# harukaki/brl

Measured on AMD Instinct MI355X. Metric: env-steps/sec at num_envs=8192, 32-step rollout, 1/2/4/8 MI355X, higher is better.
Workload: dtype u8

## Files before the change

brl_amd/csrc/brl_ppo.hip:

```cpp
#include <hip/hip_runtime.h>
#include <math.h>
#include <stdint.h>
#include <stdio.h>
#include <stdlib.h>
#include <string.h>

#include "abi_common.hpp"

static inline unsigned thread_grid(int64_t n, int bs) { return (unsigned)((n + bs - 1) / bs); }

struct PpoArgs {
  const float *logits;
  int64_t ls;
  const float *value;
  const uint8_t *mask;
  const int32_t *action;
  const float *old_value, *old_logp, *gae, *tgt;
  int64_t B;
  float clip_eps, vf_coef, ent_coef;
  int masked, value_clipping;
  float *dlogits, *dvalue, *partials, *illp;
  int64_t vs, dls, dvs;
};

// ... 297 lines not shown
  return BRL_OK;
}

#ifdef FAIR_TIMING
extern "C" int brl_fair_set_dbg(void *p) {
  HIP_TRY(hipMemcpyToSymbol(HIP_SYMBOL(g_fair_dbg), &p, sizeof(p)));
  return BRL_OK;
}
#endif

extern "C" int brl_fair_chain(int device, const brl_fair_net *net, const float *x0, const uint8_t *mask, const int32_t *action,
                              const float *old_value, const float *old_log_prob, const float *gae, const float *targets,
                              int64_t batch, float clip_eps, float vf_coef, float ent_coef, int masked, int value_clipping,
                              int reward_scaling, int act, const brl_fair_work *work, void *stream) {
  NEED(net && work && x0 && mask && action && old_value && old_log_prob && gae && targets, "NULL input");
  NEED(batch > 0 && batch % fair::R == 0, "batch (a multiple of 16)");
  NEED(act == 0 || act == 1, "act");
  fair::Args A{};
  for (int l = 0; l < 11; l++) {
    NEED(net->w[l] && net->b[l], "net: NULL layer");
    NEED((((uintptr_t)net->w[l]) & 15) == 0 && (((uintptr_t)net->b[l]) & 15) == 0, "net: 16-byte alignment");
    A.net.w[l] = net->w[l]; A.net.b[l] = net->b[l];
  }
  NEED(net->head_w && net->head_b && (((uintptr_t)net->head_w) & 15) == 0, "net: heads");
  A.net.wh = net->head_w; A.net.bh = net->head_b;
  NEED(work->inp && work->dzs && work->gates && work->cat6 && work->x4 && work->dz0 && work->dz6 && work->dheads && work->tiles &&
       work->partials, "work: NULL array");
  const void *al[] = {x0, work->inp, work->dzs, work->gates, work->cat6, work->x4, work->dz0, work->dz6, work->tiles};
  for (const void *q : al) NEED((((uintptr_t)q) & 15) == 0, "16-byte alignment");
  A.o = fair::Bufs{work->inp, work->dzs, work->gates, work->cat6, work->x4, work->dz0, work->dz6, work->dheads, work->tiles,
                   work->partials, work->gram_partials};
  A.x0 = x0;
  A.P = PpoArgs{nullptr, 0, nullptr, mask, action, old_value, old_log_prob, gae, targets, batch, clip_eps, vf_coef,
                ent_coef, masked, value_clipping, nullptr, nullptr, nullptr, nullptr, 1, BRL_NUM_ACTIONS, 1};
  A.act = act;
  A.reward_scaling = reward_scaling;
  HIP_TRY(hipSetDevice(device));
  A.nrows = batch;
  hipLaunchKernelGGL(fair::k_fair_chain<true>, dim3((unsigned)(batch / fair::R)), dim3(fair::NW * 64), 0, (hipStream_t)stream, A);
  HIP_TRY(hipGetLastError());
  return BRL_OK;
}

extern "C" int brl_fair_forward(int device, const brl_fair_net *net, const float *x, int64_t rows, int act, float *logits, float *value,
                                void *stream) {
  NEED(net && x && logits && value, "NULL array");
  NEED(rows >= 0 && rows < (1ll << 31), "rows");
  NEED(act == 0 || act == 1, "act");
  if (rows == 0) return BRL_OK;
  fair::Args A{};
  for (int l = 0; l < 11; l++) {
    NEED(net->w[l] && net->b[l], "net: NULL layer");
    NEED((((uintptr_t)net->w[l]) & 15) == 0 && (((uintptr_t)net->b[l]) & 15) == 0, "net: 16-byte alignment");
    A.net.w[l] = net->w[l]; A.net.b[l] = net->b[l];
  }
  NEED(net->head_w && net->head_b && (((uintptr_t)net->head_w) & 15) == 0 && (((uintptr_t)x) & 15) == 0, "net: heads / x: 16-byte alignment");
  A.net.wh = net->head_w; A.net.bh = net->head_b;
  A.x0 = x;
  A.act = act;
  A.nrows = rows;
  A.logits_out = logits;
  A.value_out = value;
  HIP_TRY(hipSetDevice(device));
  hipLaunchKernelGGL(fair::k_fair_chain<false>, dim3((unsigned)((rows + fair::R - 1) / fair::R)), dim3(fair::NW * 64), 0,
                     (hipStream_t)stream, A);
  HIP_TRY(hipGetLastError());
  return BRL_OK;
}

extern "C" int brl_ppo_heads_loss_split(int device, const float *h, int64_t ldh, const float *head_w, const float *head_b,
                                        int64_t hidden, const uint8_t *mask, const int32_t *action, const float *old_value,
                                        const float *old_log_prob, const float *gae, const float *targets, int64_t batch,
                                        float clip_eps, float vf_coef, float ent_coef, int masked, int value_clipping,
                                        int reward_scaling, float *heads_out, float *dheads, float *partials, float *gram_partials,
                                        float *head_parts, int ksplit, void *stream) {
  NEED(batch > 0 && hidden > 0 && hidden % 16 == 0 && ldh >= hidden && ldh % 4 == 0, "batch / hidden (a multiple of 16) / ldh");
  NEED(h && head_w && head_b && mask && action && old_value && old_log_prob && gae && targets, "NULL input array");
  NEED(dheads && partials && head_parts, "NULL output array");
  NEED(ksplit >= 1 && ksplit <= 8, "ksplit (1..8)");
// ... 170 lines not shown
```

brl_amd/csrc/fair_chain.hpp:

```cpp
#pragma once

#ifndef FAIR_EXP
#define FAIR_EXP 0
#endif
#ifdef FAIR_TIMING
__device__ unsigned long long *g_fair_dbg = nullptr;
#define FAIR_STAMP(k) do { if (threadIdx.x == 0 && g_fair_dbg) g_fair_dbg[(size_t)blockIdx.x * 64 + (k)] = __builtin_amdgcn_s_memtime(); } while (0)
#else
#define FAIR_STAMP(k) do { } while (0)
#endif
namespace fair {
constexpr int H = 200, OBS = 480, CAT = 680;
constexpr int R = 16;
constexpr int NW = 8;
constexpr int NT = 13;
constexpr int LDA = 208;
constexpr int LDX = 484;
constexpr int LDH = 48;
typedef float f32x4 __attribute__((ext_vector_type(4)));

struct Net {
  const float *w[11], *b[11];
  const float *wh, *bh;
};
struct Bufs {
  float *inp, *dzs, *gates, *cat6, *x4, *dz0, *dz6, *dheads, *tiles, *partials, *gram_partials;
};
struct Args {
// ... 12 lines not shown
__device__ __forceinline__ f32x4 act4(f32x4 v, int act) {
  if (act == 0) return f32x4{fmaxf(v.x, 0.f), fmaxf(v.y, 0.f), fmaxf(v.z, 0.f), fmaxf(v.w, 0.f)};
  return f32x4{tanhf(v.x), tanhf(v.y), tanhf(v.z), tanhf(v.w)};
}
__device__ __forceinline__ f32x4 dact4(f32x4 d, f32x4 h, int act) {
  if (act == 0) return f32x4{h.x > 0.f ? d.x : 0.f, h.y > 0.f ? d.y : 0.f, h.z > 0.f ? d.z : 0.f, h.w > 0.f ? d.w : 0.f};
  return f32x4{d.x * (1.f - h.x * h.x), d.y * (1.f - h.y * h.y), d.z * (1.f - h.z * h.z), d.w * (1.f - h.w * h.w)};
}
__device__ __forceinline__ float row16_sum(float v) {
  v += dpp_move_f<0xB1>(0.0f, v);
  v += dpp_move_f<0x4E>(0.0f, v);
  v += dpp_move_f<0x124>(0.0f, v);
  v += dpp_move_f<0x128>(0.0f, v);
  return v;
}
__device__ __forceinline__ f32x4 row16_sum4(f32x4 v) { return f32x4{row16_sum(v.x), row16_sum(v.y), row16_sum(v.z), row16_sum(v.w)}; }

constexpr int FCH = 15;
struct Frag { f32x4 w[FCH]; };
struct Job {
  const float *W;
  int ldw, nch, nn, n0, nmax;
  int real;
};

struct JobAddr {
  __amdgpu_buffer_rsrc_t rs;
  int voff, vtail;
  int nn, wide, nch;
};
__device__ __forceinline__ JobAddr job_addr(const Job &J, const int c, const int g) {
// ... 19 lines not shown
  if ((FAIR_EXP & 64) && !a.nn) return;
  if (!a.nn) {
    if (j == 12) F.w[j] = __builtin_bit_cast(f32x4, __builtin_amdgcn_raw_buffer_load_b128(a.rs, a.vtail, 0, 0));
    else F.w[j] = __builtin_bit_cast(f32x4, __builtin_amdgcn_raw_buffer_load_b128(a.rs, a.voff, 64 * j, 0));
  } else {
    const int v = (j == 12) ? a.vtail : a.voff;
    if (!a.wide) {
#pragma unroll
      for (int s = 0; s < 4; s++) F.w[j][s] = __builtin_bit_cast(float, __builtin_amdgcn_raw_buffer_load_b32(a.rs, v, (16 * j + s) * H * 4, 0));
    } else {
#pragma unroll
      for (int s = 0; s < 4; s++) F.w[j][s] = __builtin_bit_cast(float, __builtin_amdgcn_raw_buffer_load_b32(a.rs, v, (16 * j + s) * CAT * 4, 0));
    }
  }
}
template <int j>
__device__ __forceinline__ void mac_chunk(f32x4 &acc, const Frag &F, const f32x4 &xv) {
#pragma unroll
  for (int s = 0; s < 4; s++) {
    if (FAIR_EXP & 1) acc[s] += F.w[j][s] * xv[s];
    else acc = __builtin_amdgcn_mfma_f32_16x16x4f32(F.w[j][s], xv[s], acc, 0, 0, 0);
  }
}
template <int j>
__device__ __forceinline__ void slot_step(f32x4 &acc, const Frag &use, Frag &pre, const JobAddr &na, const int nch, const float *xrow,
                                          f32x4 &xv) {
  f32x4 xn = xv;
  if (!(FAIR_EXP & 4) && (j + 1 < 13 || (j + 1 < FCH && nch > 13))) xn = ld4(xrow + 16 * (j + 1));
  if (j < 13 || na.nch > 13) load_chunk<j>(pre, na);
  if (j < 13 || nch > 13) mac_chunk<j>(acc, use, xv);
  __builtin_amdgcn_sched_barrier(0);
  xv = xn;
}
__device__ __forceinline__ void slot_run(f32x4 &acc, const Frag &use, Frag &pre, const Job &cur, const Job &nxt, const float *X,
                                         const int ldx, const int c, const int g, const int gs) {
  const JobAddr na = job_addr(nxt, c, g);
  const float *xrow = X + c * ldx + 4 * (ldx == LDA ? gs : g);
  const int nch = cur.nch;
  f32x4 xv = (FAIR_EXP & 4) ? f32x4{1.f, 1.f, 1.f, 1.f} : ld4(xrow);
  __builtin_amdgcn_sched_barrier(0);
  slot_step<0>(acc, use, pre, na, nch, xrow, xv);
  slot_step<1>(acc, use, pre, na, nch, xrow, xv);
  slot_step<2>(acc, use, pre, na, nch, xrow, xv);
  slot_step<3>(acc, use, pre, na, nch, xrow, xv);
  slot_step<4>(acc, use, pre, na, nch, xrow, xv);
  slot_step<5>(acc, use, pre, na, nch, xrow, xv);
  slot_step<6>(acc, use, pre, na, nch, xrow, xv);
  slot_step<7>(acc, use, pre, na, nch, xrow, xv);
  slot_step<8>(acc, use, pre, na, nch, xrow, xv);
  slot_step<9>(acc, use, pre, na, nch, xrow, xv);
  slot_step<10>(acc, use, pre, na, nch, xrow, xv);
  slot_step<11>(acc, use, pre, na, nch, xrow, xv);
  slot_step<12>(acc, use, pre, na, nch, xrow, xv);
  if (nch > 13 || na.nch > 13) {
    slot_step<13>(acc, use, pre, na, nch, xrow, xv);
    slot_step<14>(acc, use, pre, na, nch, xrow, xv);
  }
}
__device__ __forceinline__ void load_job(Frag &F, const Job &J, const int c, const int g) {
  const JobAddr a = job_addr(J, c, g);
  load_chunk<0>(F, a); load_chunk<1>(F, a); load_chunk<2>(F, a); load_chunk<3>(F, a); load_chunk<4>(F, a); load_chunk<5>(F, a);
  load_chunk<6>(F, a); load_chunk<7>(F, a); load_chunk<8>(F, a); load_chunk<9>(F, a); load_chunk<10>(F, a); load_chunk<11>(F, a);
  load_chunk<12>(F, a);
  if (a.nch > 13) { load_chunk<13>(F, a); load_chunk<14>(F, a); }
}

template <bool TRAIN>
__global__ __launch_bounds__(NW * 64) void k_fair_chain(Args A) {
  __shared__ __attribute__((aligned(16))) float X0[R * LDX];
  __shared__ __attribute__((aligned(16))) float AB[3][R * LDA];
  __shared__ __attribute__((aligned(16))) float HD[R * LDH], DH[TRAIN ? R * LDH : 4];
  __shared__ float illp_s[TRAIN ? R : 1][BRL_NUM_ACTIONS], part_s[TRAIN ? R : 1][8];
  __shared__ float rs_red[NW], rs_stat[2];
  const int tid = (int)threadIdx.x, lane = tid & 63, c = lane & 15, g = lane >> 4;
  const int gs = g ^ ((0x78 >> (2 * (c >> 2))) & 3);
  const int sw4 = 4 * (gs - g);
  const int w = __builtin_amdgcn_readfirstlane(tid >> 6);
  const int64_t B = TRAIN ? A.P.B : A.nrows, row0 = (int64_t)blockIdx.x * R, nwg = gridDim.x;
  const int act = A.act;
  const Net &N = A.net;
  const Bufs &O = A.o;
  const int64_t BH = B * H;
  float *const a0 = AB[0], *const a1 = AB[1], *const a2 = AB[2];

  const bool hasA = w < 7, hasB = w < 6;
  const int tA = hasA ? 32 * w : 0, tB = hasB ? tA + 16 : tA;
  auto job_fwd = [&](const float *W, int ldw, int nch, bool B) { return Job{W, ldw, nch, 0, B ? tB : tA, H, (B ? hasB : hasA) ? 1 : 0}; };
  auto job_bwd = [&](const float *W, int ldw, bool B) { return Job{W, ldw, 13, 1, B ? tB : tA, H, (B ? hasB : hasA) ? 1 : 0}; };
  Frag FP, FQ;
  int stamp_i = 0;
  (void)stamp_i;
  FAIR_STAMP(stamp_i++);
  constexpr int XP = (R * (OBS / 4) + NW * 64 - 1) / (NW * 64);
  f32x4 xv[XP];
#pragma unroll
  for (int i = 0; i < XP; i++) {
    const int e = tid + i * NW * 64, ec = (e < R * (OBS / 4)) ? e : 0;
    const int r = ec / (OBS / 4), q = ec - r * (OBS / 4);
// ... 37 lines not shown
    q = wave_sum_f(q);
    __syncthreads();
    if (lane == 0) rs_red[w] = q;
    __syncthreads();
    if (tid == 0) {
      float t = 0.0f;
      for (int k = 0; k < NW; k++) t += rs_red[k];
      rs_stat[1] = 1.0f / (sqrtf(t / (float)B) + 1e-8f);
    }
    __syncthreads();
    adv_inv = rs_stat[1];
  }
  __syncthreads();
  FAIR_STAMP(stamp_i++);

  const int64_t grow = (row0 + c) * H;
  float *const sink = AB[0];
  auto gptr = [&](float *base, int col) { return (FAIR_EXP & 8) ? sink + c * LDA + (col % 200) : base + grow + col; };
  const f32x4 zero4 = f32x4{0.f, 0.f, 0.f, 0.f};
  auto gst = [&](float *p, const f32x4 &v) { if (TRAIN) st4(p, v); };

  auto slot = [&](Frag &use, Frag &pre, const Job &cur, const Job &nxt, const float *X, int ldx, f32x4 &acc, const float *e4) {
    const f32x4 e = ld4(e4);
    slot_run(acc, use, pre, cur, nxt, X, ldx, c, g, gs);
    return e;
  };
  struct E2 { f32x4 a, b; };
  auto slot2 = [&](Frag &use, Frag &pre, const Job &cur, const Job &nxt, const float *X, int ldx, f32x4 &acc, const float *e4a,
                   const float *e4b) {
    E2 e;
    e.a = ld4(e4a);
    e.b = ld4(e4b);
    slot_run(acc, use, pre, cur, nxt, X, ldx, c, g, gs);
    return e;
  };
  auto colc = [&](int n0) { const int col = n0 + 4 * g; return (col < H) ? col : H - 4; };
  auto phase200 = [&](Frag &F1, Frag &F2, const Job &jA, const Job &jB, const float *X, const Job &next, auto &&eptr, auto &&ep) {
    f32x4 acc = zero4;
    f32x4 e = slot(F1, F2, jA, jB, X, LDA, acc, eptr(jA.n0));
    ep(acc, e, jA.n0, hasA);
    acc = zero4;
    e = slot(F2, F1, jB, next, X, LDA, acc, eptr(jB.n0));
    ep(acc, e, jB.n0, hasB);
    __syncthreads();
    FAIR_STAMP(stamp_i++);
  };
  auto fwd_jobs = [&](int l, Job &jA, Job &jB) {
    jA = job_fwd(N.w[l], H, 13, false);
    jB = job_fwd(N.w[l], H, 13, true);
  };
  auto bwd_jobs = [&](int l, int ldw, Job &jA, Job &jB) {
    jA = job_bwd(N.w[l], ldw, false);
    jB = job_bwd(N.w[l], ldw, true);
  };

  {
    auto ep = [&](const f32x4 &acc, const f32x4 &bias, int n0, bool valid) {
      const int col = n0 + 4 * g;
      if (col < H && valid) {
        const f32x4 z = acc + bias, h = act4(z, act);
        st4(a0 + c * LDA + col + sw4, z);
        st4(a1 + c * LDA + col + sw4, h);
        gst(gptr(O.inp + 0 * BH, col), h);
      }
    };
    const Job jA0 = job_fwd(N.w[0], OBS, 15, false), jA1 = job_fwd(N.w[0] + 240, OBS, 15, false);
    const Job jB0 = job_fwd(N.w[0], OBS, 15, true), jB1 = job_fwd(N.w[0] + 240, OBS, 15, true);
    f32x4 acc = zero4;
    f32x4 e = slot(FP, FQ, jA0, jA1, X0, LDX, acc, N.b[0] + colc(tA));
    (void)slot(FQ, FP, jA1, jB0, X0 + 240, LDX, acc, N.b[0]);
    ep(acc, e, tA, hasA);
    acc = zero4;
    e = slot(FP, FQ, jB0, jB1, X0, LDX, acc, N.b[0] + colc(tB));
    (void)slot(FQ, FP, jB1, job_fwd(N.w[1], H, 13, false), X0 + 240, LDX, acc, N.b[0]);
    ep(acc, e, tB, hasB);
    __syncthreads();
    FAIR_STAMP(stamp_i++);
  }
  auto layer = [&](const float *in, float *out, int l, float *gout, const Job &next) {
    Job jA, jB;
    fwd_jobs(l, jA, jB);
    phase200(FP, FQ, jA, jB, in, next, [&](int n0) { return N.b[l] + colc(n0); },
             [&](const f32x4 &acc, const f32x4 &bias, int n0, bool valid) {
      const int col = n0 + 4 * g;
      if (col < H && valid) {
        const f32x4 h = act4(acc + bias, act);
        st4(out + c * LDA + col + sw4, h);
        gst(gptr(gout, col), h);
      }
    });
  };
  auto layer_res = [&](const float *in, float *res, int l, float *ggate, float *out, float *gout, bool act_out, const Job &next) {
    Job jA, jB;
    fwd_jobs(l, jA, jB);
    phase200(FP, FQ, jA, jB, in, next, [&](int n0) { return N.b[l] + colc(n0); },
             [&](const f32x4 &acc, const f32x4 &bias, int n0, bool valid) {
      const int col = n0 + 4 * g;
      if (col < H && valid) {
        const f32x4 h = act4(acc + bias, act);
        gst(gptr(ggate, col), h);
        const f32x4 x = h + ld4(res + c * LDA + col + sw4);
        st4(res + c * LDA + col + sw4, x);
        if (act_out) {
          const f32x4 gg = act4(x, act);
          st4(out + c * LDA + col + sw4, gg);
          gst(gptr(gout, col), gg);
        } else {
          gst(gptr(gout, col), x);
        }
      }
    });
  };
  auto first_fwd = [&](int l) { return job_fwd(N.w[l], H, 13, false); };
  layer(a1, a2, 1, O.inp + 1 * BH, first_fwd(2));
  layer_res(a2, a0, 2, O.gates + 0 * BH, a1, O.inp + 2 * BH, true, first_fwd(3));
  layer(a1, a2, 3, O.inp + 3 * BH, first_fwd(4));
  layer_res(a2, a0, 4, O.gates + 1 * BH, nullptr, O.inp + 4 * BH, false, first_fwd(5));
  {
    Job jA, jB;
    fwd_jobs(5, jA, jB);
    phase200(FP, FQ, jA, jB, a0, job_fwd(N.w[6], CAT, 13, false), [&](int n0) { return N.b[5] + colc(n0); },
             [&](const f32x4 &acc, const f32x4 &bias, int n0, bool valid) {
      const int col = n0 + 4 * g;
      if (col < H && valid) {
        const f32x4 z = acc + bias;
        st4(a1 + c * LDA + col + sw4, z);
        gst(O.cat6 + (row0 + c) * CAT + col, z);
      }
    });
  }
  {
    auto ep = [&](const f32x4 &acc, const f32x4 &bias, int n0, bool valid) {
      const int col = n0 + 4 * g;
      if (col < H && valid) {
        const f32x4 z = acc + bias, h = act4(z, act);
        st4(a0 + c * LDA + col + sw4, z);
        st4(a2 + c * LDA + col + sw4, h);
        gst(gptr(O.inp + 5 * BH, col), h);
      }
    };
    const float *W6 = N.w[6];
    const Job jA0 = job_fwd(W6, CAT, 13, false), jA1 = job_fwd(W6 + H, CAT, 15, false), jA2 = job_fwd(W6 + H + 240, CAT, 15, false);
    const Job jB0 = job_fwd(W6, CAT, 13, true), jB1 = job_fwd(W6 + H, CAT, 15, true), jB2 = job_fwd(W6 + H + 240, CAT, 15, true);
    f32x4 acc = zero4;
    f32x4 e = slot(FP, FQ, jA0, jA1, a1, LDA, acc, N.b[6] + colc(tA));
    (void)slot(FQ, FP, jA1, jA2, X0, LDX, acc, N.b[6]);
    (void)slot(FP, FQ, jA2, jB0, X0 + 240, LDX, acc, N.b[6]);
    ep(acc, e, tA, hasA);
    acc = zero4;
    e = slot(FQ, FP, jB0, jB1, a1, LDA, acc, N.b[6] + colc(tB));
    (void)slot(FP, FQ, jB1, jB2, X0, LDX, acc, N.b[6]);
    (void)slot(FQ, FP, jB2, first_fwd(7), X0 + 240, LDX, acc, N.b[6]);
    ep(acc, e, tB, hasB);
    __syncthreads();
    FAIR_STAMP(stamp_i++);
  }
  layer(a2, a1, 7, O.inp + 6 * BH, first_fwd(8));
  layer_res(a1, a0, 8, O.gates + 2 * BH, a2, O.inp + 7 * BH, true, first_fwd(9));
  layer(a2, a1, 9, O.inp + 8 * BH, first_fwd(10));
  const Job jheads = Job{N.wh, H, 13, 0, 16 * ((w < 3) ? w : 2), HD_NOUT, (w < 3) ? 1 : 0};
  PpoSampleIn smp[2];
  if (TRAIN) {
    smp[0] = ppo_sample_load(A.P, row0 + 2 * w, true, lane);
    smp[1] = ppo_sample_load(A.P, row0 + 2 * w + 1, true, lane);
  }
  layer_res(a1, a0, 10, O.gates + 3 * BH, nullptr, O.x4, false, jheads);
  {
    Job bA, bB;
    bwd_jobs(10, H, bA, bB);
    (void)bB;
    if (!TRAIN) bA.real = 0;
    f32x4 acc = zero4;
    (void)slot(FP, FQ, jheads, bA, a0, LDA, acc, N.b[0]);
    if (w < 3) {
      const int col = 16 * w + 4 * g;
#pragma unroll
      for (int i = 0; i < 4; i++)
        if (col + i < HD_NOUT) HD[c * LDH + col + i] = acc[i] + N.bh[col + i];
    }
    __syncthreads();
    FAIR_STAMP(stamp_i++);
  }

  if (!TRAIN) {
    for (int e = tid; e < R * HD_NOUT; e += NW * 64) {
      const int r = e / HD_NOUT, n = e - r * HD_NOUT;
      if (row0 + r < B) {
        if (n < BRL_NUM_ACTIONS) A.logits_out[(row0 + r) * BRL_NUM_ACTIONS + n] = HD[r * LDH + n];
        else A.value_out[row0 + r] = HD[r * LDH + n];
      }
    }
    return;
  }

  f32x4 hw_[2][3], hg_[2];
  {
    const float *g3 = O.gates + 3 * BH;
#pragma unroll
    for (int i = 0; i < 2; i++) {
      const int t = (w + 8 * i < NT) ? w + 8 * i : w, n = (16 * t + c < H) ? 16 * t + c : H - 1;
#pragma unroll
      for (int j = 0; j < 3; j++) {
#pragma unroll
        for (int q = 0; q < 4; q++) {
          const int k = 16 * j + 4 * g + q;
          hw_[i][j][q] = N.wh[(int64_t)((k < HD_NOUT) ? k : HD_NOUT - 1) * H + n];
        }
      }
      hg_[i] = ld4(g3 + grow + colc(16 * t));
    }
  }

  {
    PpoArgs P = A.P;
    P.dlogits = DH; P.dls = LDH; P.dvalue = DH + BRL_NUM_ACTIONS; P.dvs = LDH; P.illp = &illp_s[0][0];
#pragma unroll
    for (int i = 0; i < 2; i++) {
      const int r = 2 * w + i;
      const PpoSampleIn S = smp[i];
      const float lg = (lane < HD_NOUT) ? HD[r * LDH + lane] : 0.0f;
      const float v = HD[r * LDH + BRL_NUM_ACTIONS];
      const float adv = A.reward_scaling ? (S.gae - adv_mean) * adv_inv : S.gae;
      float st[5], ill;
      ppo_loss_sample(P, S, r, true, lane, lg, v, adv, st, ill);
      if (lane == 0) {
#pragma unroll
        for (int k = 0; k < 8; k++) part_s[r][k] = (k < 5) ? st[k] : 0.0f;
      }
    }
  }
  __syncthreads();
  FAIR_STAMP(stamp_i++);
  if (tid < 8) {
// ... 10 lines not shown
      O.gram_partials[(int64_t)blockIdx.x * HD_GRAM + e] = s;
    }
  }
  for (int e = tid; e < R * 40; e += NW * 64) {
    const int r = e / 40, n = e - r * 40;
    O.dheads[(row0 + r) * 40 + n] = DH[r * LDH + n];
  }
  float *const tiles_wg = O.tiles + (int64_t)blockIdx.x * H;
  const int64_t tstride = nwg * H;
  if (tid < HD_NOUT) {
    float s = 0.0f;
    for (int r = 0; r < R; r++) s += DH[r * LDH + tid];
    O.tiles[11 * tstride + (int64_t)blockIdx.x * HD_NOUT + tid] = s;
  }

  auto colsum = [&](f32x4 v, int col, int l) {
    const f32x4 s = row16_sum4(v);
    if (c == 0 && col < H) st4(tiles_wg + l * tstride + col, s);
  };
  struct Then { const float *gate2; float *dst2, *gout2; int lsum2; };
  auto then_step = [&](const f32x4 &dx, const f32x4 &g2, int col, bool valid, const Then &T) {
    f32x4 v = zero4;
    if (col < H && valid) {
      v = (T.gate2 != nullptr) ? dact4(dx, g2, act) : dx;
      if (T.dst2 != nullptr) st4(T.dst2 + c * LDA + col + sw4, v);
      st4(gptr(T.gout2, col), v);
    }
    if (valid) colsum(v, col, T.lsum2);
  };
  {
    const Then T{O.gates + 3 * BH, a1, O.dzs + 8 * BH, 10};
#pragma unroll
    for (int i = 0; i < 2; i++) {
      const bool valid = w + 8 * i < NT;
      const int t = valid ? w + 8 * i : w, col = 16 * t + 4 * g;
      f32x4 acc = zero4;
#pragma unroll
      for (int j = 0; j < 3; j++) {
        const f32x4 xv = ld4(DH + c * LDH + 16 * j + 4 * g);
#pragma unroll
        for (int q = 0; q < 4; q++) acc = __builtin_amdgcn_mfma_f32_16x16x4f32(hw_[i][j][q], xv[q], acc, 0, 0, 0);
      }
      if (col < H && valid) st4(a0 + c * LDA + col + sw4, acc);
      then_step(acc, hg_[i], col, valid, T);
    }
    __syncthreads();
    FAIR_STAMP(stamp_i++);
  }
  auto back = [&](const float *src, float *dst, int l, int ldw, const float *ggate, float *gout, int lsum, bool accumulate,
                  const Job &next, const Then *T) {
    Job jA, jB;
    bwd_jobs(l, ldw, jA, jB);
    const float *gbase = (ggate != nullptr) ? ggate : O.inp;
    const float *g2base = (T != nullptr && T->gate2 != nullptr) ? T->gate2 : O.inp;
    auto ep = [&](const f32x4 &acc, const E2 &e, int n0, bool valid) {
      const int col = n0 + 4 * g;
      f32x4 v = zero4;
      if (col < H && valid) {
        v = acc;
        if (ggate != nullptr) v = dact4(v, e.a, act);
        if (accumulate) v += ld4(dst + c * LDA + col + sw4);
        st4(dst + c * LDA + col + sw4, v);
        if (gout != nullptr) st4(gptr(gout, col), v);
      }
      if (lsum >= 0 && valid) colsum(v, col, lsum);
      if (T != nullptr) then_step(v, e.b, col, valid, *T);
    };
    f32x4 acc = zero4;
    E2 e = slot2(FQ, FP, jA, jB, src, LDA, acc, gbase + grow + colc(jA.n0), g2base + grow + colc(jA.n0));
    ep(acc, e, jA.n0, hasA);
    acc = zero4;
    e = slot2(FP, FQ, jB, next, src, LDA, acc, gbase + grow + colc(jB.n0), g2base + grow + colc(jB.n0));
    ep(acc, e, jB.n0, hasB);
    __syncthreads();
    FAIR_STAMP(stamp_i++);
  };
  auto first_bwd = [&](int l, int ldw) { return job_bwd(N.w[l], ldw, false); };
  auto block = [&](int lb, int la, int ia, const float *ga, const float *gin, const Job &next, const Then &T, float *zb, float *za) {
    back(zb, za, lb, H, ga, O.dzs + (int64_t)ia * BH, la, false, first_bwd(la, H), nullptr);
    back(za, a0, la, H, gin, nullptr, -1, true, next, &T);
  };
  const Then T8{O.gates + 2 * BH, a1, O.dzs + 6 * BH, 8}, T6{nullptr, nullptr, O.dz6, 6}, T4{O.gates + 1 * BH, a2, O.dzs + 3 * BH, 4},
      T2{O.gates + 0 * BH, a2, O.dzs + 1 * BH, 2}, T0{nullptr, nullptr, O.dz0, 0};
  block(10, 9, 7, O.inp + 8 * BH, O.inp + 7 * BH, first_bwd(8, H), T8, a1, a2);
  block(8, 7, 5, O.inp + 6 * BH, O.inp + 5 * BH, first_bwd(6, CAT), T6, a1, a2);
  back(a0, a1, 6, CAT, nullptr, O.dzs + 4 * BH, 5, false, first_bwd(5, H), nullptr);
  back(a1, a0, 5, H, nullptr, nullptr, -1, false, first_bwd(4, H), &T4);
// ... 5 lines not shown
```

brl_amd/fused_update.py:

```python
from __future__ import annotations

import torch
import torch.distributed as dist

from ._capture import quiet_gc
from .roll_out import Transition


_CAPTURE_GROUP = {}


def _capture_group():
    key = dist.get_world_size(), dist.get_rank()
    if key not in _CAPTURE_GROUP:
        g = dist.new_group(backend="nccl")
        try:
            dev = torch.device("cuda", torch.cuda.current_device())
            g._get_backend(dev).eager_connect_single_device(dev)
        except Exception:
            pass
        _CAPTURE_GROUP[key] = g
    return _CAPTURE_GROUP[key]


# ... 574 lines not shown
        torch.mm(self.dzs[0].t(), self.x0, out=self.GW[0])

    def _seg_fin(self):
        self.capi.check(self.lib.brl_bias_finalize_ex(self._di(), self._nseg, self._seg_scratch, self._seg_cols, self._seg_tiles,
                                                      self._seg_db, torch.cuda.current_stream().cuda_stream))

    def _fin_opt(self):
        self.capi.check(self.lib.brl_adam_clip_fin_gather(
            self._di(), self.P.data_ptr(), self.G.data_ptr(), self.M.data_ptr(), self.V.data_ptr(), self.n, self.step.data_ptr(), self.lr,
            self.lr_dev.data_ptr(), float(self.b1), float(self.b2), self.eps, self.max_norm, self.scratch.data_ptr(),
            self.scratch.numel(), self.mb_index.data_ptr(), self.norm.data_ptr(), self.gargs.data_ptr(), self.mbs, self._nseg,
            self._seg_scratch, self._seg_cols, self._seg_tiles, self._seg_db, torch.cuda.current_stream().cuda_stream))



class FusedFair(FusedStep):

    SQUARE = (1, 2, 3, 4, 5, 7, 8, 9, 10)
    INPUT = {1: "h0", 2: "h1", 3: "g1", 4: "h3", 5: "x2", 7: "h6", 8: "h7", 9: "g3", 10: "h9"}

    @staticmethod
    def supports(config, params) -> bool:
        return (bool(config.get("fused_update", True)) and getattr(params, "model", "") == "FAIR"
                and getattr(params, "act", None) in (torch.relu, torch.tanh)
                and next(params.parameters()).is_cuda and next(params.parameters()).dtype == torch.float32)

    def _layout(self):
        p = self.params
        L = list(p.l)
        plist = [L[l].weight for l in self.SQUARE] + [L[0].weight, L[6].weight, p.actor.weight, p.critic.weight] \
# ... 32 lines not shown
        self.ones_row = torch.ones((1, B), dtype=torch.float32, device=self.dev)
        self.unit_gate = torch.ones((B, H), dtype=torch.float32, device=self.dev) if self.act == 0 else f(B, H)
        self.own_gemm = bool(self.cfg.get("own_gemm", True)) and B % 4 == 0 and H % 4 == 0
        self.from_gemm = (1, 3, 7, 9) if self.own_gemm else ()
        t16, t64 = (B + 15) // 16, (B + 63) // 64
        self.tiles = [f((t64 if l in self.from_gemm else t16), H) for l in range(11)]
        self._seg_scratch = (C.c_void_p * 11)(*[t.data_ptr() for t in self.tiles])
        self._seg_cols = (C.c_int64 * 11)(*([H] * 11))
        self._seg_tiles = (C.c_int64 * 11)(*[t.shape[0] for t in self.tiles])
        self._seg_db = (C.c_void_p * 11)(*[g.data_ptr() for g in self.Gb])
        if not self.multi:
            g = self.capi.ShardGeom()
            g.nbuckets, g.world, g.nsub = 1, 1, 1024
            g.off[0], g.len[0] = 0, self.n
            self.geom, self.norm_partials = g, f(1024)
        self.chain = bool(self.cfg.get("fair_chain", True)) and B % 16 == 0 and H == 200 and self.x0.shape[1] == 480 and not self.ill_coef
        if self.ill_coef:
            self.heads39, self.dheads39, self.vec = f(B, 39), f(B, 39), f(40)
        if self.chain:
            nwg = B // 16
            assert p.critic.weight.data_ptr() == p.actor.weight.data_ptr() + 38 * H * 4 \
                and p.critic.bias.data_ptr() == p.actor.bias.data_ptr() + 38 * 4
            sw, sb = views[p.actor.weight], views[p.critic.bias]
            self.GWh = self.G[sw.start:sw.start + 39 * H].view(39, H)
            self.gates, self.dheads = f(4, B, H), f(B, 40)
            self.ctiles = f(11 * nwg * H + nwg * 39)
            self.cpartials, self.cgram = f(nwg, 8), f(nwg, 38 * 38)
            net, wk = self.capi.FairNet(), self.capi.FairWork()
            for l, lin in enumerate(L):
                net.w[l], net.b[l] = lin.weight.data_ptr(), lin.bias.data_ptr()
            net.head_w, net.head_b = p.actor.weight.data_ptr(), p.actor.bias.data_ptr()
            for name, t_ in (("inp", self.inp), ("dzs", self.dzs), ("gates", self.gates), ("cat6", self.cat6), ("x4", self.t["x4"]),
                             ("dz0", self.dz[0]), ("dz6", self.dz[6]), ("dheads", self.dheads), ("tiles", self.ctiles),
                             ("partials", self.cpartials), ("gram_partials", self.cgram)):
                setattr(wk, name, t_.data_ptr())
# ... 163 lines not shown
```

Before: 10.70 billion.

## Run training chain kernel with 4 rows per workgroup using 4x4x1 MFMA

```diff
diff --git a/brl_amd/csrc/brl_ppo.hip b/brl_amd/csrc/brl_ppo.hip
--- a/brl_amd/csrc/brl_ppo.hip
+++ b/brl_amd/csrc/brl_ppo.hip
@@ -335,7 +335,7 @@
                               int64_t batch, float clip_eps, float vf_coef, float ent_coef, int masked, int value_clipping,
                               int reward_scaling, int act, const brl_fair_work *work, void *stream) {
   NEED(net && work && x0 && mask && action && old_value && old_log_prob && gae && targets, "NULL input");
-  NEED(batch > 0 && batch % fair::R == 0, "batch (a multiple of 16)");
+  NEED(batch > 0 && batch % fair::R_STEP == 0, "batch (a multiple of 4)");
   NEED(act == 0 || act == 1, "act");
   fair::Args A{};
   for (int l = 0; l < 11; l++) {
@@ -358,7 +358,8 @@
   A.reward_scaling = reward_scaling;
   HIP_TRY(hipSetDevice(device));
   A.nrows = batch;
-  hipLaunchKernelGGL(fair::k_fair_chain<true>, dim3((unsigned)(batch / fair::R)), dim3(fair::NW * 64), 0, (hipStream_t)stream, A);
+  hipLaunchKernelGGL((fair::k_fair_chain<true, fair::R_STEP>), dim3((unsigned)(batch / fair::R_STEP)), dim3(fair::NW * 64), 0,
+                     (hipStream_t)stream, A);
   HIP_TRY(hipGetLastError());
   return BRL_OK;
 }
@@ -383,7 +384,7 @@
   A.logits_out = logits;
   A.value_out = value;
   HIP_TRY(hipSetDevice(device));
-  hipLaunchKernelGGL(fair::k_fair_chain<false>, dim3((unsigned)((rows + fair::R - 1) / fair::R)), dim3(fair::NW * 64), 0,
+  hipLaunchKernelGGL((fair::k_fair_chain<false, fair::R_FWD>), dim3((unsigned)((rows + fair::R_FWD - 1) / fair::R_FWD)), dim3(fair::NW * 64), 0,
                      (hipStream_t)stream, A);
   HIP_TRY(hipGetLastError());
   return BRL_OK;
diff --git a/brl_amd/csrc/fair_chain.hpp b/brl_amd/csrc/fair_chain.hpp
--- a/brl_amd/csrc/fair_chain.hpp
+++ b/brl_amd/csrc/fair_chain.hpp
@@ -2,6 +2,9 @@
 
 #ifndef FAIR_EXP
 #define FAIR_EXP 0
+#endif
+#ifndef FAIR_STEP_ROWS
+#define FAIR_STEP_ROWS 4
 #endif
 #ifdef FAIR_TIMING
 __device__ unsigned long long *g_fair_dbg = nullptr;
@@ -11,7 +14,9 @@
 #endif
 namespace fair {
 constexpr int H = 200, OBS = 480, CAT = 680;
-constexpr int R = 16;
+constexpr int R_STEP = FAIR_STEP_ROWS;
+constexpr int R_FWD = 16;
+static_assert(R_STEP == 4 || R_STEP == 8, "FAIR_STEP_ROWS: 4 or 8");
 constexpr int NW = 8;
 constexpr int NT = 13;
 constexpr int LDA = 208;
@@ -54,7 +59,18 @@
   v += dpp_move_f<0x128>(0.0f, v);
   return v;
 }
-__device__ __forceinline__ f32x4 row16_sum4(f32x4 v) { return f32x4{row16_sum(v.x), row16_sum(v.y), row16_sum(v.z), row16_sum(v.w)}; }
+__device__ __forceinline__ float quad_sum(float v) {
+  v += dpp_move_f<0xB1>(0.0f, v);
+  v += dpp_move_f<0x4E>(0.0f, v);
+  return v;
+}
+__device__ __forceinline__ float ksum(float v) {
+  const auto p = __builtin_amdgcn_permlane32_swap(__float_as_uint(v), __float_as_uint(v), false, false);
+  v = __uint_as_float(p[0]) + __uint_as_float(p[1]);
+  const auto q = __builtin_amdgcn_permlane16_swap(__float_as_uint(v), __float_as_uint(v), false, false);
+  return __uint_as_float(q[0]) + __uint_as_float(q[1]);
+}
+__device__ __forceinline__ f32x4 ksum4(f32x4 v) { return f32x4{ksum(v.x), ksum(v.y), ksum(v.z), ksum(v.w)}; }
 
 constexpr int FCH = 15;
 struct Frag { f32x4 w[FCH]; };
@@ -104,48 +120,64 @@
     }
   }
 }
-template <int j>
-__device__ __forceinline__ void mac_chunk(f32x4 &acc, const Frag &F, const f32x4 &xv) {
+template <int j, int RG, bool M16>
+__device__ __forceinline__ void mac_chunk(f32x4 (&acc)[RG], const Frag &F, const f32x4 (&xv)[RG]) {
 #pragma unroll
   for (int s = 0; s < 4; s++) {
-    if (FAIR_EXP & 1) acc[s] += F.w[j][s] * xv[s];
-    else acc = __builtin_amdgcn_mfma_f32_16x16x4f32(F.w[j][s], xv[s], acc, 0, 0, 0);
-  }
-}
-template <int j>
-__device__ __forceinline__ void slot_step(f32x4 &acc, const Frag &use, Frag &pre, const JobAddr &na, const int nch, const float *xrow,
-                                          f32x4 &xv) {
-  f32x4 xn = xv;
-  if (!(FAIR_EXP & 4) && (j + 1 < 13 || (j + 1 < FCH && nch > 13))) xn = ld4(xrow + 16 * (j + 1));
+#pragma unroll
+    for (int rg = 0; rg < RG; rg++) {
+      if (FAIR_EXP & 1) acc[rg][s] += F.w[j][s] * xv[rg][s];
+      else if (M16) acc[rg] = __builtin_amdgcn_mfma_f32_16x16x4f32(F.w[j][s], xv[rg][s], acc[rg], 0, 0, 0);
+      else acc[rg] = __builtin_amdgcn_mfma_f32_4x4x1f32(F.w[j][s], xv[rg][s], acc[rg], 0, 0, 0);
+    }
+  }
+}
+template <int j, int RG, bool M16>
+__device__ __forceinline__ void slot_step(f32x4 (&acc)[RG], const Frag &use, Frag &pre, const JobAddr &na, const int nch,
+                                          const float *const (&xrow)[RG], f32x4 (&xv)[RG]) {
+  f32x4 xn[RG];
+#pragma unroll
+  for (int rg = 0; rg < RG; rg++) {
+    xn[rg] = xv[rg];
+    if (!(FAIR_EXP & 4) && (j + 1 < 13 || (j + 1 < FCH && nch > 13))) xn[rg] = ld4(xrow[rg] + 16 * (j + 1));
+  }
   if (j < 13 || na.nch > 13) load_chunk<j>(pre, na);
-  if (j < 13 || nch > 13) mac_chunk<j>(acc, use, xv);
+  if (j < 13 || nch > 13) mac_chunk<j, RG, M16>(acc, use, xv);
   __builtin_amdgcn_sched_barrier(0);
-  xv = xn;
-}
-__device__ __forceinline__ void slot_run(f32x4 &acc, const Frag &use, Frag &pre, const Job &cur, const Job &nxt, const float *X,
-                                         const int ldx, const int c, const int g, const int gs) {
+#pragma unroll
+  for (int rg = 0; rg < RG; rg++) xv[rg] = xn[rg];
+}
+template <int RG, bool M16>
+__device__ __forceinline__ void slot_run(f32x4 (&acc)[RG], const Frag &use, Frag &pre, const Job &cur, const Job &nxt,
+                                         const float *const (&xrow)[RG], const int c, const int g) {
   const JobAddr na = job_addr(nxt, c, g);
-  const float *xrow = X + c * ldx + 4 * (ldx == LDA ? gs : g);
   const int nch = cur.nch;
-  f32x4 xv = (FAIR_EXP & 4) ? f32x4{1.f, 1.f, 1.f, 1.f} : ld4(xrow);
+  f32x4 xv[RG], p[RG];
+#pragma unroll
+  for (int rg = 0; rg < RG; rg++) {
+    xv[rg] = (FAIR_EXP & 4) ? f32x4{1.f, 1.f, 1.f, 1.f} : ld4(xrow[rg]);
+    p[rg] = M16 ? acc[rg] : f32x4{0.f, 0.f, 0.f, 0.f};
+  }
   __builtin_amdgcn_sched_barrier(0);
-  slot_step<0>(acc, use, pre, na, nch, xrow, xv);
-  slot_step<1>(acc, use, pre, na, nch, xrow, xv);
-  slot_step<2>(acc, use, pre, na, nch, xrow, xv);
-  slot_step<3>(acc, use, pre, na, nch, xrow, xv);
-  slot_step<4>(acc, use, pre, na, nch, xrow, xv);
-  slot_step<5>(acc, use, pre, na, nch, xrow, xv);
-  slot_step<6>(acc, use, pre, na, nch, xrow, xv);
-  slot_step<7>(acc, use, pre, na, nch, xrow, xv);
-  slot_step<8>(acc, use, pre, na, nch, xrow, xv);
-  slot_step<9>(acc, use, pre, na, nch, xrow, xv);
-  slot_step<10>(acc, use, pre, na, nch, xrow, xv);
-  slot_step<11>(acc, use, pre, na, nch, xrow, xv);
-  slot_step<12>(acc, use, pre, na, nch, xrow, xv);
+  slot_step<0, RG, M16>(p, use, pre, na, nch, xrow, xv);
+  slot_step<1, RG, M16>(p, use, pre, na, nch, xrow, xv);
+  slot_step<2, RG, M16>(p, use, pre, na, nch, xrow, xv);
+  slot_step<3, RG, M16>(p, use, pre, na, nch, xrow, xv);
+  slot_step<4, RG, M16>(p, use, pre, na, nch, xrow, xv);
+  slot_step<5, RG, M16>(p, use, pre, na, nch, xrow, xv);
+  slot_step<6, RG, M16>(p, use, pre, na, nch, xrow, xv);
+  slot_step<7, RG, M16>(p, use, pre, na, nch, xrow, xv);
+  slot_step<8, RG, M16>(p, use, pre, na, nch, xrow, xv);
+  slot_step<9, RG, M16>(p, use, pre, na, nch, xrow, xv);
+  slot_step<10, RG, M16>(p, use, pre, na, nch, xrow, xv);
+  slot_step<11, RG, M16>(p, use, pre, na, nch, xrow, xv);
+  slot_step<12, RG, M16>(p, use, pre, na, nch, xrow, xv);
   if (nch > 13 || na.nch > 13) {
-    slot_step<13>(acc, use, pre, na, nch, xrow, xv);
-    slot_step<14>(acc, use, pre, na, nch, xrow, xv);
-  }
+    slot_step<13, RG, M16>(p, use, pre, na, nch, xrow, xv);
+    slot_step<14, RG, M16>(p, use, pre, na, nch, xrow, xv);
+  }
+#pragma unroll
+  for (int rg = 0; rg < RG; rg++) acc[rg] = M16 ? p[rg] : acc[rg] + ksum4(p[rg]);
 }
 __device__ __forceinline__ void load_job(Frag &F, const Job &J, const int c, const int g) {
   const JobAddr a = job_addr(J, c, g);
@@ -155,16 +187,22 @@
   if (a.nch > 13) { load_chunk<13>(F, a); load_chunk<14>(F, a); }
 }
 
-template <bool TRAIN>
+template <bool TRAIN, int R>
 __global__ __launch_bounds__(NW * 64) void k_fair_chain(Args A) {
+  static_assert(R == 4 || R == 8 || R == 16, "rows per workgroup");
+  constexpr bool M16 = R == 16;
+  constexpr int RG = M16 ? 1 : R / 4;
+  constexpr int RPW = (R + NW - 1) / NW;
   __shared__ __attribute__((aligned(16))) float X0[R * LDX];
   __shared__ __attribute__((aligned(16))) float AB[3][R * LDA];
   __shared__ __attribute__((aligned(16))) float HD[R * LDH], DH[TRAIN ? R * LDH : 4];
   __shared__ float illp_s[TRAIN ? R : 1][BRL_NUM_ACTIONS], part_s[TRAIN ? R : 1][8];
   __shared__ float rs_red[NW], rs_stat[2];
   const int tid = (int)threadIdx.x, lane = tid & 63, c = lane & 15, g = lane >> 4;
-  const int gs = g ^ ((0x78 >> (2 * (c >> 2))) & 3);
-  const int sw4 = 4 * (gs - g);
+  const int gs = M16 ? g ^ ((0x78 >> (2 * (c >> 2))) & 3) : g;
+  const int lcol = M16 ? 4 * g : 4 * (c >> 2);
+  const int sw4 = M16 ? 4 * (gs - g) : 0;
+  const bool own = M16 || g == 0;
   const int w = __builtin_amdgcn_readfirstlane(tid >> 6);
   const int64_t B = TRAIN ? A.P.B : A.nrows, row0 = (int64_t)blockIdx.x * R, nwg = gridDim.x;
   const int act = A.act;
@@ -172,6 +210,7 @@
   const Bufs &O = A.o;
   const int64_t BH = B * H;
   float *const a0 = AB[0], *const a1 = AB[1], *const a2 = AB[2];
+  auto rowof = [&](int rg) { return M16 ? c : 4 * rg + (c & 3); };
 
   const bool hasA = w < 7, hasB = w < 6;
   const int tA = hasA ? 32 * w : 0, tB = hasB ? tA + 16 : tA;
@@ -239,32 +278,48 @@
   __syncthreads();
   FAIR_STAMP(stamp_i++);
 
-  const int64_t grow = (row0 + c) * H;
   float *const sink = AB[0];
-  auto gptr = [&](float *base, int col) { return (FAIR_EXP & 8) ? sink + c * LDA + (col % 200) : base + grow + col; };
+  auto gptr = [&](float *base, int row, int col) {
+    return (FAIR_EXP & 8) ? sink + row * LDA + (col % 200) : base + (row0 + row) * H + col;
+  };
+  auto lds = [&](float *buf, int row, int col) { return buf + row * LDA + col + sw4; };
   const f32x4 zero4 = f32x4{0.f, 0.f, 0.f, 0.f};
   auto gst = [&](float *p, const f32x4 &v) { if (TRAIN) st4(p, v); };
-
-  auto slot = [&](Frag &use, Frag &pre, const Job &cur, const Job &nxt, const float *X, int ldx, f32x4 &acc, const float *e4) {
+  auto xrows = [&](const float *X, int ldx, const float *(&xr)[RG]) {
+    for (int rg = 0; rg < RG; rg++) xr[rg] = X + rowof(rg) * ldx + 4 * (ldx == LDA ? gs : g);
+  };
+
+  auto slot = [&](Frag &use, Frag &pre, const Job &cur, const Job &nxt, const float *X, int ldx, f32x4 (&acc)[RG], const float *e4) {
     const f32x4 e = ld4(e4);
-    slot_run(acc, use, pre, cur, nxt, X, ldx, c, g, gs);
+    const float *xr[RG];
+    xrows(X, ldx, xr);
+    slot_run<RG, M16>(acc, use, pre, cur, nxt, xr, c, g);
     return e;
   };
-  struct E2 { f32x4 a, b; };
-  auto slot2 = [&](Frag &use, Frag &pre, const Job &cur, const Job &nxt, const float *X, int ldx, f32x4 &acc, const float *e4a,
-                   const float *e4b) {
+  struct E2 { f32x4 a[RG], b[RG]; };
+  auto slot2 = [&](Frag &use, Frag &pre, const Job &cur, const Job &nxt, const float *X, int ldx, f32x4 (&acc)[RG], const float *ga,
+                   const float *gb, int col) {
     E2 e;
-    e.a = ld4(e4a);
-    e.b = ld4(e4b);
-    slot_run(acc, use, pre, cur, nxt, X, ldx, c, g, gs);
+#pragma unroll
+    for (int rg = 0; rg < RG; rg++) {
+      e.a[rg] = ld4(ga + (row0 + rowof(rg)) * H + col);
+      e.b[rg] = ld4(gb + (row0 + rowof(rg)) * H + col);
+    }
+    const float *xr[RG];
+    xrows(X, ldx, xr);
+    slot_run<RG, M16>(acc, use, pre, cur, nxt, xr, c, g);
     return e;
   };
-  auto colc = [&](int n0) { const int col = n0 + 4 * g; return (col < H) ? col : H - 4; };
+  auto zero_acc = [&](f32x4 (&acc)[RG]) {
+    for (int rg = 0; rg < RG; rg++) acc[rg] = zero4;
+  };
+  auto colc = [&](int n0) { const int col = n0 + lcol; return (col < H) ? col : H - 4; };
   auto phase200 = [&](Frag &F1, Frag &F2, const Job &jA, const Job &jB, const float *X, const Job &next, auto &&eptr, auto &&ep) {
-    f32x4 acc = zero4;
+    f32x4 acc[RG];
+    zero_acc(acc);
     f32x4 e = slot(F1, F2, jA, jB, X, LDA, acc, eptr(jA.n0));
     ep(acc, e, jA.n0, hasA);
-    acc = zero4;
+    zero_acc(acc);
     e = slot(F2, F1, jB, next, X, LDA, acc, eptr(jB.n0));
     ep(acc, e, jB.n0, hasB);
     __syncthreads();
@@ -280,22 +335,27 @@
   };
 
   {
-    auto ep = [&](const f32x4 &acc, const f32x4 &bias, int n0, bool valid) {
-      const int col = n0 + 4 * g;
-      if (col < H && valid) {
-        const f32x4 z = acc + bias, h = act4(z, act);
-        st4(a0 + c * LDA + col + sw4, z);
-        st4(a1 + c * LDA + col + sw4, h);
-        gst(gptr(O.inp + 0 * BH, col), h);
+    auto ep = [&](const f32x4 (&acc)[RG], const f32x4 &bias, int n0, bool valid) {
+      const int col = n0 + lcol;
+      if (col < H && valid && own) {
+#pragma unroll
+        for (int rg = 0; rg < RG; rg++) {
+          const int row = rowof(rg);
+          const f32x4 z = acc[rg] + bias, h = act4(z, act);
+          st4(lds(a0, row, col), z);
+          st4(lds(a1, row, col), h);
+          gst(gptr(O.inp + 0 * BH, row, col), h);
+        }
       }
     };
     const Job jA0 = job_fwd(N.w[0], OBS, 15, false), jA1 = job_fwd(N.w[0] + 240, OBS, 15, false);
     const Job jB0 = job_fwd(N.w[0], OBS, 15, true), jB1 = job_fwd(N.w[0] + 240, OBS, 15, true);
-    f32x4 acc = zero4;
+    f32x4 acc[RG];
+    zero_acc(acc);
     f32x4 e = slot(FP, FQ, jA0, jA1, X0, LDX, acc, N.b[0] + colc(tA));
     (void)slot(FQ, FP, jA1, jB0, X0 + 240, LDX, acc, N.b[0]);
     ep(acc, e, tA, hasA);
-    acc = zero4;
+    zero_acc(acc);
     e = slot(FP, FQ, jB0, jB1, X0, LDX, acc, N.b[0] + colc(tB));
     (void)slot(FQ, FP, jB1, job_fwd(N.w[1], H, 13, false), X0 + 240, LDX, acc, N.b[0]);
     ep(acc, e, tB, hasB);
@@ -306,12 +366,16 @@
     Job jA, jB;
     fwd_jobs(l, jA, jB);
     phase200(FP, FQ, jA, jB, in, next, [&](int n0) { return N.b[l] + colc(n0); },
-             [&](const f32x4 &acc, const f32x4 &bias, int n0, bool valid) {
-      const int col = n0 + 4 * g;
-      if (col < H && valid) {
-        const f32x4 h = act4(acc + bias, act);
-        st4(out + c * LDA + col + sw4, h);
-        gst(gptr(gout, col), h);
+             [&](const f32x4 (&acc)[RG], const f32x4 &bias, int n0, bool valid) {
+      const int col = n0 + lcol;
+      if (col < H && valid && own) {
+#pragma unroll
+        for (int rg = 0; rg < RG; rg++) {
+          const int row = rowof(rg);
+          const f32x4 h = act4(acc[rg] + bias, act);
+          st4(lds(out, row, col), h);
+          gst(gptr(gout, row, col), h);
+        }
       }
     });
   };
@@ -319,19 +383,23 @@
     Job jA, jB;
     fwd_jobs(l, jA, jB);
     phase200(FP, FQ, jA, jB, in, next, [&](int n0) { return N.b[l] + colc(n0); },
-             [&](const f32x4 &acc, const f32x4 &bias, int n0, bool valid) {
-      const int col = n0 + 4 * g;
-      if (col < H && valid) {
-        const f32x4 h = act4(acc + bias, act);
-        gst(gptr(ggate, col), h);
-        const f32x4 x = h + ld4(res + c * LDA + col + sw4);
-        st4(res + c * LDA + col + sw4, x);
-        if (act_out) {
-          const f32x4 gg = act4(x, act);
-          st4(out + c * LDA + col + sw4, gg);
-          gst(gptr(gout, col), gg);
-        } else {
-          gst(gptr(gout, col), x);
+             [&](const f32x4 (&acc)[RG], const f32x4 &bias, int n0, bool valid) {
+      const int col = n0 + lcol;
+      if (col < H && valid && own) {
+#pragma unroll
+        for (int rg = 0; rg < RG; rg++) {
+          const int row = rowof(rg);
+          const f32x4 h = act4(acc[rg] + bias, act);
+          gst(gptr(ggate, row, col), h);
+          const f32x4 x = h + ld4(lds(res, row, col));
+          st4(lds(res, row, col), x);
+          if (act_out) {
+            const f32x4 gg = act4(x, act);
+            st4(lds(out, row, col), gg);
+            gst(gptr(gout, row, col), gg);
+          } else {
+            gst(gptr(gout, row, col), x);
+          }
         }
       }
     });
@@ -345,34 +413,43 @@
     Job jA, jB;
     fwd_jobs(5, jA, jB);
     phase200(FP, FQ, jA, jB, a0, job_fwd(N.w[6], CAT, 13, false), [&](int n0) { return N.b[5] + colc(n0); },
-             [&](const f32x4 &acc, const f32x4 &bias, int n0, bool valid) {
-      const int col = n0 + 4 * g;
-      if (col < H && valid) {
-        const f32x4 z = acc + bias;
-        st4(a1 + c * LDA + col + sw4, z);
-        gst(O.cat6 + (row0 + c) * CAT + col, z);
+             [&](const f32x4 (&acc)[RG], const f32x4 &bias, int n0, bool valid) {
+      const int col = n0 + lcol;
+      if (col < H && valid && own) {
+#pragma unroll
+        for (int rg = 0; rg < RG; rg++) {
+          const int row = rowof(rg);
+          const f32x4 z = acc[rg] + bias;
+          st4(lds(a1, row, col), z);
+          gst(O.cat6 + (row0 + row) * CAT + col, z);
+        }
       }
     });
   }
   {
-    auto ep = [&](const f32x4 &acc, const f32x4 &bias, int n0, bool valid) {
-      const int col = n0 + 4 * g;
-      if (col < H && valid) {
-        const f32x4 z = acc + bias, h = act4(z, act);
-        st4(a0 + c * LDA + col + sw4, z);
-        st4(a2 + c * LDA + col + sw4, h);
-        gst(gptr(O.inp + 5 * BH, col), h);
+    auto ep = [&](const f32x4 (&acc)[RG], const f32x4 &bias, int n0, bool valid) {
+      const int col = n0 + lcol;
+      if (col < H && valid && own) {
+#pragma unroll
+        for (int rg = 0; rg < RG; rg++) {
+          const int row = rowof(rg);
+          const f32x4 z = acc[rg] + bias, h = act4(z, act);
+          st4(lds(a0, row, col), z);
+          st4(lds(a2, row, col), h);
+          gst(gptr(O.inp + 5 * BH, row, col), h);
+        }
       }
     };
     const float *W6 = N.w[6];
     const Job jA0 = job_fwd(W6, CAT, 13, false), jA1 = job_fwd(W6 + H, CAT, 15, false), jA2 = job_fwd(W6 + H + 240, CAT, 15, false);
     const Job jB0 = job_fwd(W6, CAT, 13, true), jB1 = job_fwd(W6 + H, CAT, 15, true), jB2 = job_fwd(W6 + H + 240, CAT, 15, true);
-    f32x4 acc = zero4;
+    f32x4 acc[RG];
+    zero_acc(acc);
     f32x4 e = slot(FP, FQ, jA0, jA1, a1, LDA, acc, N.b[6] + colc(tA));
     (void)slot(FQ, FP, jA1, jA2, X0, LDX, acc, N.b[6]);
     (void)slot(FP, FQ, jA2, jB0, X0 + 240, LDX, acc, N.b[6]);
     ep(acc, e, tA, hasA);
-    acc = zero4;
+    zero_acc(acc);
     e = slot(FQ, FP, jB0, jB1, a1, LDA, acc, N.b[6] + colc(tB));
     (void)slot(FP, FQ, jB1, jB2, X0, LDX, acc, N.b[6]);
     (void)slot(FQ, FP, jB2, first_fwd(7), X0 + 240, LDX, acc, N.b[6]);
@@ -384,10 +461,11 @@
   layer_res(a1, a0, 8, O.gates + 2 * BH, a2, O.inp + 7 * BH, true, first_fwd(9));
   layer(a2, a1, 9, O.inp + 8 * BH, first_fwd(10));
   const Job jheads = Job{N.wh, H, 13, 0, 16 * ((w < 3) ? w : 2), HD_NOUT, (w < 3) ? 1 : 0};
-  PpoSampleIn smp[2];
+  PpoSampleIn smp[RPW];
   if (TRAIN) {
-    smp[0] = ppo_sample_load(A.P, row0 + 2 * w, true, lane);
-    smp[1] = ppo_sample_load(A.P, row0 + 2 * w + 1, true, lane);
+#pragma unroll
+    for (int i = 0; i < RPW; i++)
+      if (RPW * w + i < R) smp[i] = ppo_sample_load(A.P, row0 + RPW * w + i, true, lane);
   }
   layer_res(a1, a0, 10, O.gates + 3 * BH, nullptr, O.x4, false, jheads);
   {
@@ -395,13 +473,17 @@
     bwd_jobs(10, H, bA, bB);
     (void)bB;
     if (!TRAIN) bA.real = 0;
-    f32x4 acc = zero4;
+    f32x4 acc[RG];
+    zero_acc(acc);
     (void)slot(FP, FQ, jheads, bA, a0, LDA, acc, N.b[0]);
-    if (w < 3) {
-      const int col = 16 * w + 4 * g;
-#pragma unroll
-      for (int i = 0; i < 4; i++)
-        if (col + i < HD_NOUT) HD[c * LDH + col + i] = acc[i] + N.bh[col + i];
+    if (w < 3 && own) {
+      const int col = 16 * w + lcol;
+#pragma unroll
+      for (int rg = 0; rg < RG; rg++) {
+#pragma unroll
+        for (int i = 0; i < 4; i++)
+          if (col + i < HD_NOUT) HD[rowof(rg) * LDH + col + i] = acc[rg][i] + N.bh[col + i];
+      }
     }
     __syncthreads();
     FAIR_STAMP(stamp_i++);
@@ -418,7 +500,7 @@
     return;
   }
 
-  f32x4 hw_[2][3], hg_[2];
+  f32x4 hw_[2][3], hg_[2][RG];
   {
     const float *g3 = O.gates + 3 * BH;
 #pragma unroll
@@ -432,7 +514,8 @@
           hw_[i][j][q] = N.wh[(int64_t)((k < HD_NOUT) ? k : HD_NOUT - 1) * H + n];
         }
       }
-      hg_[i] = ld4(g3 + grow + colc(16 * t));
+#pragma unroll
+      for (int rg = 0; rg < RG; rg++) hg_[i][rg] = ld4(g3 + (row0 + rowof(rg)) * H + colc(16 * t));
     }
   }
 
@@ -440,8 +523,9 @@
     PpoArgs P = A.P;
     P.dlogits = DH; P.dls = LDH; P.dvalue = DH + BRL_NUM_ACTIONS; P.dvs = LDH; P.illp = &illp_s[0][0];
 #pragma unroll
-    for (int i = 0; i < 2; i++) {
-      const int r = 2 * w + i;
+    for (int i = 0; i < RPW; i++) {
+      const int r = RPW * w + i;
+      if (r >= R) continue;
       const PpoSampleIn S = smp[i];
       const float lg = (lane < HD_NOUT) ? HD[r * LDH + lane] : 0.0f;
       const float v = HD[r * LDH + BRL_NUM_ACTIONS];
@@ -482,17 +566,26 @@
     O.tiles[11 * tstride + (int64_t)blockIdx.x * HD_NOUT + tid] = s;
   }
 
-  auto colsum = [&](f32x4 v, int col, int l) {
-    const f32x4 s = row16_sum4(v);
-    if (c == 0 && col < H) st4(tiles_wg + l * tstride + col, s);
+  auto colsum = [&](const f32x4 (&v)[RG], int col, int l) {
+    f32x4 s = v[0];
+#pragma unroll
+    for (int rg = 1; rg < RG; rg++) s += v[rg];
+    s = M16 ? f32x4{row16_sum(s.x), row16_sum(s.y), row16_sum(s.z), row16_sum(s.w)}
+            : f32x4{quad_sum(s.x), quad_sum(s.y), quad_sum(s.z), quad_sum(s.w)};
+    if ((M16 ? c == 0 : (c & 3) == 0 && g == 0) && col < H) st4(tiles_wg + l * tstride + col, s);
   };
   struct Then { const float *gate2; float *dst2, *gout2; int lsum2; };
-  auto then_step = [&](const f32x4 &dx, const f32x4 &g2, int col, bool valid, const Then &T) {
-    f32x4 v = zero4;
-    if (col < H && valid) {
-      v = (T.gate2 != nullptr) ? dact4(dx, g2, act) : dx;
-      if (T.dst2 != nullptr) st4(T.dst2 + c * LDA + col + sw4, v);
-      st4(gptr(T.gout2, col), v);
+  auto then_step = [&](const f32x4 (&dx)[RG], const f32x4 (&g2)[RG], int col, bool valid, const Then &T) {
+    f32x4 v[RG];
+#pragma unroll
+    for (int rg = 0; rg < RG; rg++) {
+      v[rg] = zero4;
+      if (col < H && valid && own) {
+        const int row = rowof(rg);
+        v[rg] = (T.gate2 != nullptr) ? dact4(dx[rg], g2[rg], act) : dx[rg];
+        if (T.dst2 != nullptr) st4(lds(T.dst2, row, col), v[rg]);
+        st4(gptr(T.gout2, row, col), v[rg]);
+      }
     }
     if (valid) colsum(v, col, T.lsum2);
   };
@@ -501,15 +594,26 @@
 #pragma unroll
     for (int i = 0; i < 2; i++) {
       const bool valid = w + 8 * i < NT;
-      const int t = valid ? w + 8 * i : w, col = 16 * t + 4 * g;
-      f32x4 acc = zero4;
+      const int t = valid ? w + 8 * i : w, col = 16 * t + lcol;
+      f32x4 acc[RG];
+      zero_acc(acc);
 #pragma unroll
       for (int j = 0; j < 3; j++) {
-        const f32x4 xv = ld4(DH + c * LDH + 16 * j + 4 * g);
-#pragma unroll
-        for (int q = 0; q < 4; q++) acc = __builtin_amdgcn_mfma_f32_16x16x4f32(hw_[i][j][q], xv[q], acc, 0, 0, 0);
-      }
-      if (col < H && valid) st4(a0 + c * LDA + col + sw4, acc);
+#pragma unroll
+        for (int rg = 0; rg < RG; rg++) {
+          const f32x4 xv = ld4(DH + rowof(rg) * LDH + 16 * j + 4 * g);
+#pragma unroll
+          for (int q = 0; q < 4; q++) {
+            if (M16) acc[rg] = __builtin_amdgcn_mfma_f32_16x16x4f32(hw_[i][j][q], xv[q], acc[rg], 0, 0, 0);
+            else acc[rg] = __builtin_amdgcn_mfma_f32_4x4x1f32(hw_[i][j][q], xv[q], acc[rg], 0, 0, 0);
+          }
+        }
+      }
+#pragma unroll
+      for (int rg = 0; rg < RG; rg++) {
+        if (!M16) acc[rg] = ksum4(acc[rg]);
+        if (col < H && valid && own) st4(lds(a0, rowof(rg), col), acc[rg]);
+      }
       then_step(acc, hg_[i], col, valid, T);
     }
     __syncthreads();
@@ -521,24 +625,30 @@
     bwd_jobs(l, ldw, jA, jB);
     const float *gbase = (ggate != nullptr) ? ggate : O.inp;
     const float *g2base = (T != nullptr && T->gate2 != nullptr) ? T->gate2 : O.inp;
-    auto ep = [&](const f32x4 &acc, const E2 &e, int n0, bool valid) {
-      const int col = n0 + 4 * g;
-      f32x4 v = zero4;
-      if (col < H && valid) {
-        v = acc;
-        if (ggate != nullptr) v = dact4(v, e.a, act);
-        if (accumulate) v += ld4(dst + c * LDA + col + sw4);
-        st4(dst + c * LDA + col + sw4, v);
-        if (gout != nullptr) st4(gptr(gout, col), v);
+    auto ep = [&](const f32x4 (&acc)[RG], const E2 &e, int n0, bool valid) {
+      const int col = n0 + lcol;
+      f32x4 v[RG];
+#pragma unroll
+      for (int rg = 0; rg < RG; rg++) {
+        v[rg] = zero4;
+        if (col < H && valid && own) {
+          const int row = rowof(rg);
+          v[rg] = acc[rg];
+          if (ggate != nullptr) v[rg] = dact4(v[rg], e.a[rg], act);
+          if (accumulate) v[rg] += ld4(lds(dst, row, col));
+          st4(lds(dst, row, col), v[rg]);
+          if (gout != nullptr) st4(gptr(gout, row, col), v[rg]);
+        }
       }
       if (lsum >= 0 && valid) colsum(v, col, lsum);
       if (T != nullptr) then_step(v, e.b, col, valid, *T);
     };
-    f32x4 acc = zero4;
-    E2 e = slot2(FQ, FP, jA, jB, src, LDA, acc, gbase + grow + colc(jA.n0), g2base + grow + colc(jA.n0));
+    f32x4 acc[RG];
+    zero_acc(acc);
+    E2 e = slot2(FQ, FP, jA, jB, src, LDA, acc, gbase, g2base, colc(jA.n0));
     ep(acc, e, jA.n0, hasA);
-    acc = zero4;
-    e = slot2(FP, FQ, jB, next, src, LDA, acc, gbase + grow + colc(jB.n0), g2base + grow + colc(jB.n0));
+    zero_acc(acc);
+    e = slot2(FP, FQ, jB, next, src, LDA, acc, gbase, g2base, colc(jB.n0));
     ep(acc, e, jB.n0, hasB);
     __syncthreads();
     FAIR_STAMP(stamp_i++);
diff --git a/brl_amd/fused_update.py b/brl_amd/fused_update.py
--- a/brl_amd/fused_update.py
+++ b/brl_amd/fused_update.py
@@ -612,6 +612,9 @@
 
 
 
+FAIR_CHAIN_ROWS = 4
+
+
 class FusedFair(FusedStep):
 
     SQUARE = (1, 2, 3, 4, 5, 7, 8, 9, 10)
@@ -674,11 +677,11 @@
             g.nbuckets, g.world, g.nsub = 1, 1, 1024
             g.off[0], g.len[0] = 0, self.n
             self.geom, self.norm_partials = g, f(1024)
-        self.chain = bool(self.cfg.get("fair_chain", True)) and B % 16 == 0 and H == 200 and self.x0.shape[1] == 480 and not self.ill_coef
+        self.chain = bool(self.cfg.get("fair_chain", True)) and B % FAIR_CHAIN_ROWS == 0 and H == 200 and self.x0.shape[1] == 480 and not self.ill_coef
         if self.ill_coef:
             self.heads39, self.dheads39, self.vec = f(B, 39), f(B, 39), f(40)
         if self.chain:
-            nwg = B // 16
+            nwg = B // FAIR_CHAIN_ROWS
             assert p.critic.weight.data_ptr() == p.actor.weight.data_ptr() + 38 * H * 4 \
                 and p.critic.bias.data_ptr() == p.actor.bias.data_ptr() + 38 * 4
             sw, sb = views[p.actor.weight], views[p.critic.bias]
```

Result: no change. 10.64 billion (median of 2 runs) (-0.5%).
